# vivek87799/lightweight-human-pose-estimation.pytorch

Measured on AMD Instinct MI355X. Metric: frames/sec end-to-end (net+grouping) at 368px, higher is better.
Workload: dtype f32; 1 GPU; batch=1 per GPU, 368x656 frames, 1 refinement stage(s), fp32 convs / f32+f64 post, resident normalised NCHW input -> key-points + pose entries on host; 3 frame batch(es) in flight per GPU (3 engine stream(s), each step a complete pass); global_batch=1, parallelism=dp1 (frames sharded, no data-path collective), 3 stream(s) per GPU

## Files before the change

### lightweight-human-pose-estimation.pytorch_amd/csrc/capi.cpp

```cpp
#include <algorithm>
#include <cmath>
#include <cstdio>
#include <cstdlib>
#include <cstring>
#include <map>
#include <mutex>
#include <string>
#include <system_error>
#include <thread>
#include <vector>

#include "jpeg_host.h"
#include "lwp_internal.h"
#include "lwp_owners.h"

using namespace lwp;

struct lwp_context {
    int device = 0;
    Stream stream, post_own;
    hipStream_t post_stream = nullptr;
    int dtype = LWP_F32;
    Graph g;
    Tuning tune;
// ... 720 lines not shown
}
static inline int buf_level(const lwp_context* h, int buf) {
    const int nb = (int)h->g.bufs.size();
    return buf < 0 ? 0 : buf < nb ? h->g.bufs[buf].level : h->tp.bufs[buf - nb].level;
}

static int enqueue_layer(lwp_context* h, const Layer& l, const float* d_in, int N, int H, int W, float* const* d_outs_nchw,
                         const Layer* fold = nullptr, bool* folded = nullptr) {
    const bool h16 = h->dtype != LWP_F32;
    const int f16 = h->dtype == LWP_F16;
    const float* wts = h->blob(l.w_off);
    const float* bias = h->blob(l.b_off);
    int dh, dw;
    level_dims(H, W, buf_level(h, l.dst.buf), &dh, &dw);
    float* dst = buf_at(h, l.dst);
    char* vb = h->record_variants ? h->variant_buf : nullptr;
    if (vb) vb[0] = 0;
    if (l.kind == L_STEM) {
        StemParams p{d_in, wts, bias, dst, N, H, W, dh, dw, f16, h->d_zeros.as<float>()};
        p.tune = &h->tune; p.variant = vb;
        LAUNCH(h, KC_STEM, h16 ? launch_stem_bf16(p, h->stream) : launch_stem(p, h->stream));
    } else if (l.kind == L_DWPW) {
        int sh, sw;
        level_dims(H, W, buf_level(h, l.src.buf), &sh, &sw);
        DwPwParams p;
        p.in = buf_at(h, l.src); p.in_ld = l.src.ld; p.f16 = f16;
        p.dw_w = wts; p.pw_w = h->blob(l.w2_off); p.pw_b = h->blob(l.b2_off);
        p.out = dst; p.out_ld = l.dst.ld;
        p.res = l.res.buf >= 0 ? buf_at(h, l.res) : nullptr; p.res_ld = l.res.ld;
        p.zeros = h->d_zeros.as<float>();
        p.N = N; p.Hi = sh; p.Wi = sw; p.Ho = dh; p.Wo = dw; p.C = l.cin; p.cout = l.cout;
        p.stride = l.stride; p.dil = l.dil; p.act_dw = l.act; p.act_pw = l.act2;
        p.tune = &h->tune; p.variant = vb;
        LAUNCH(h, KC_PW, h16 ? launch_dwpw_bf16(p, h->stream) : launch_dwpw(p, h->stream));
    } else if (l.kind == L_DW) {
        int sh, sw;
        level_dims(H, W, buf_level(h, l.src.buf), &sh, &sw);
        DwParams p{buf_at(h, l.src), l.src.ld, wts, bias, dst, l.dst.ld, N, sh, sw, dh, dw, l.cin, l.stride, l.dil, l.act};
        p.tune = &h->tune; p.variant = vb;
        LAUNCH(h, KC_DW, launch_dw(p, h->stream));
    } else {
        GemmParams p;
        p.in = buf_at(h, l.src); p.in_ld = l.src.ld; p.f16 = f16;
        p.w = wts; p.bias = bias;
        p.wf = h16 ? nullptr : h->blob(l.w2_off);
        p.out = dst; p.out_ld = l.dst.ld;
        p.res = l.res.buf >= 0 ? buf_at(h, l.res) : nullptr; p.res_ld = l.res.ld;
        p.out_nchw = (l.out_index >= 0 && d_outs_nchw) ? d_outs_nchw[l.out_index] : nullptr;
        p.out_nchw2 = (l.out_index2 >= 0 && d_outs_nchw) ? d_outs_nchw[l.out_index2] : nullptr;
        p.out_split = l.out_split;
        p.zeros = h->d_zeros.as<float>();
        p.N = N; p.H = dh; p.W = dw;
        p.cin_pad = l.cin_pad; p.cout = l.cout; p.cout_pad = l.cout_pad; p.ks = l.ks; p.dil = l.dil; p.act = l.act;
        p.tune = &h->tune; p.variant = vb;
        if (fold) {
            p.w2 = h->blob(fold->w_off); p.bias2 = h->blob(fold->b_off);
            p.out2 = buf_at(h, fold->dst); p.out2_ld = fold->dst.ld; p.act2 = fold->act;
            p.fused2 = folded;
        }
        LAUNCH(h, l.ks == 1 ? KC_PW : KC_C3, h16 ? launch_gemm_bf16(p, h->stream) : launch_gemm(p, h->stream));
    }
    if (vb && h->cur_layer >= 0 && h->cur_layer < (int)h->variants.size()) h->variants[h->cur_layer] = vb;
    return LWP_OK;
}

static bool heads_pair_runs(const lwp_context* h, const Layer& a, const Layer& b, int64_t M) {
// ... 33 lines not shown
    return LWP_OK;
}

static int enqueue_forward(lwp_context* h, const std::vector<Layer>& ls, int begin, int end, const float* d_in, int N, int H, int W,
                           float* const* d_outs_nchw, bool retain = false) {
    int fh, fw;
    level_dims(H, W, 3, &fh, &fw);
    const int64_t M3 = (int64_t)N * fh * fw;
    int rc = LWP_OK;
    for (int i = begin; i < end && rc == LWP_OK; ++i) {
        h->cur_layer = i;
        const bool inside = i + 1 < end;
        if (inside && heads_pair_runs(h, ls[i], ls[i + 1], M3)) {
            if (retain) rc = enqueue_layer(h, ls[i], d_in, N, H, W, nullptr);
            if (!rc) rc = enqueue_heads_pair(h, ls[i], ls[i + 1], N, H, W, d_outs_nchw);
            ++i;
            continue;
        }
        if (retain && &ls == &h->tp.layers) {
            if (h->tp.dw_copy[i] >= 0) {
                rc = enqueue_dw_copy(h, ls[i], h->tp.dw_copy[i], N, H, W);
                if (rc) break;
            }
            if (h->tp.nores_copy[i] >= 0) {
                Layer c = ls[i];
                c.res = BufRef();
                c.dst.buf = h->tp.nores_copy[i]; c.dst.coff = 0;
                c.out_index = c.out_index2 = -1;
                rc = enqueue_layer(h, c, d_in, N, H, W, nullptr);
                if (rc) break;
            }
        }
        bool folded = false;
        rc = enqueue_layer(h, ls[i], d_in, N, H, W, d_outs_nchw, inside && ls[i].fuse == LWP_MARK_FOLD_NEXT_1X1 ? &ls[i + 1] : nullptr, &folded);
        if (!rc && folded) {
            if (h->record_variants && (size_t)i + 1 < h->variants.size()) h->variants[i + 1] = h->variants[i];
            ++i;
        }
    }
    h->cur_layer = -1;
    return rc;
}
static int enqueue_network(lwp_context* h, const float* d_in, int N, int H, int W, float* const* d_outs_nchw) {
    return enqueue_forward(h, h->g.layers, 0, (int)h->g.layers.size(), d_in, N, H, W, d_outs_nchw);
}

static int check_frame_shape(lwp_context* h, int N, int H, int W) {
    if (N <= 0 || H <= 0 || W <= 0) return fail(h, LWP_ERR_ARG, "bad frame shape");
    if (H < 8 || W < 8) return fail(h, LWP_ERR_ARG, "frame too small (H, W >= 8)");
    if (!h->weights_loaded) return fail(h, LWP_ERR_STATE, "weights not loaded (call lwp_load_weights first)");
    return LWP_OK;
}

static int stage_input(lwp_context* h, const float* in, int in_mem, size_t bytes, const float** d_in) {
    if (in_mem == LWP_MEM_DEVICE) { *d_in = in; return LWP_OK; }
    HIP_TRY(h, h->d_in.ensure(bytes));
    HIP_TRY(h, hipMemcpyAsync(h->d_in.as<float>(), in, bytes, hipMemcpyHostToDevice, h->stream));
    *d_in = h->d_in.as<float>();
    return LWP_OK;
}

extern "C" int lwp_forward(lwp_handle h, const float* in, int in_mem, int N, int H, int W, float* const* outs, int out_mem) {
    if (!h || !in || !outs) return fail(h, LWP_ERR_ARG, "null argument");
    int rc = check_frame_shape(h, N, H, W);
    if (rc) return rc;
    HIP_TRY(h, hipSetDevice(h->device));
    rc = ensure_activations(h, frames_per_pass(h, N, H, W), H, W);
    if (rc) return rc;
    if (in_mem == LWP_MEM_DEVICE || out_mem == LWP_MEM_DEVICE) { rc = order_in(h); if (rc) return rc; }
// ... 3948 lines not shown
```

### lightweight-human-pose-estimation.pytorch_amd/csrc/lwp_internal.h

```cpp
#pragma once
#include <hip/hip_runtime.h>
#include <stdint.h>
#include <algorithm>
#include <cstdio>
#include <string>
#include <vector>

#include "../../include/lwpose.h"

namespace lwp {

struct ParamSpec {
    std::string key;
    int64_t shape[4];
    int ndim;
    int role;
};
std::vector<ParamSpec> param_table(int nref, int C, int NH, int NP);

enum LayerKind { L_STEM = 0, L_DW = 1, L_GEMM = 2, L_DWPW = 3 };
enum Act { ACT_NONE = 0, ACT_RELU = 1, ACT_ELU = 2 };
enum KClass { KC_STEM = 0, KC_DW = 1, KC_PW = 2, KC_C3 = 3, KC_POST = 4, KC_OTHER = 5, KC_COUNT = 6 };

struct BufRef {
    int buf = -1;
    int coff = 0;
    int ld = 0;
};

struct WBlock {
    std::string conv_key;
    int out_off, in_off, cout, cin;
};

struct Layer {
    int kind = L_GEMM;
    std::string name;
    std::string conv_key;
    std::string bn_key;
    bool has_bias = false;
    int cin = 0, cout = 0, ks = 1, stride = 1, dil = 1, act = ACT_NONE;
    BufRef src, dst, res;
    int out_index = -1;
    int out_index2 = -1, out_split = 0;
    std::vector<WBlock> blocks;
    int64_t macs_per_pixel = 0;
    int fuse = LWP_MARK_NONE;
    size_t w_off = 0, b_off = 0;
    int cin_pad = 0, cout_pad = 0;
    std::string conv2_key, bn2_key;
    int act2 = ACT_NONE;
    size_t w2_off = 0, b2_off = 0;
};

struct BufSpec {
    int level;
    int channels;
    bool has_pad = false;
};

struct Graph {
    int nref, C, NH, NP;
    std::vector<BufSpec> bufs;
    std::vector<Layer> layers;
    size_t blob_floats = 0;
    int cat_buf = -1;
    int cat_channels = 0;
    int dtype = LWP_F32;
};
Graph build_graph(int nref, int C, int NH, int NP, bool fuse_dwpw, int dtype, bool merge_heads = true);

struct TrainPlan {
    std::vector<Layer> layers;
    std::vector<BufSpec> bufs;
    std::vector<int> cats;
    int cpm_conv = -1;
    int cpm_in = -1;
    int cut = -1;
    std::vector<int> dw_copy, nores_copy;
    enum { GRAD_ALWAYS = 0, GRAD_NEVER = 1, GRAD_ON_DEMAND = 2 };
    std::vector<char> grad_mode;
};
TrainPlan build_train_plan(const Graph& g, int scope = LWP_TRAIN_STAGES);
uint16_t f32_to_f16_rne(float f);
uint16_t f32_to_bf16_rne(float f);

struct HostTensor {
    const void* ptr;
    int64_t shape[4];
    int ndim;
};
std::string pack_weights(const Graph& g, const std::vector<std::string>& names,
                         const std::vector<HostTensor>& tensors, std::vector<float>& blob);

struct Tuning {
    int stem_ty = 0, stem_wl = -1, stem_debug = 0;
    int dw_tiled = -1, dw_cc = 0, dw_ph = 0;
    int dw_px = 0;
    int gemm_wp = -1;
    int gemm_debug = 0;
    bool has_c3 = false, has_pw = false; int c3[3] = {0, 0, 0}, pw[3] = {0, 0, 0};
    int dwpw_bm = 0, dwpw_nw = 0, dwpw_debug = 0, dwpwh_debug = 0;
    int dwpw_pipe = -1;
    int dwpw_lean = -1;
    int dwpw_tiled_wgs = 0;
    int dwpw_tiled = -1;
    int dwpw_pp_grid = 0;
    int dwpw_pp = -1;
    int heads_rm = 0;
    int gemmh_fold = -1;
    int gemmh_persist = -1, gemmh_ar_off = 0, gemmh_ar_force = 0, gemmh_debug = 0;
    bool has_gemmh_ar = false, has_gemmh = false; int gemmh_ar[4] = {0, 0, 0, 0}, gemmh[4] = {0, 0, 0, 0};
    int upsample_tiled = -1;
    int max_frames_per_pass = 0;
    int peak_tile = -1, pair_form = -1;
    int dwpw_lds_pad_kb = 0;
    int host_fetch_dma = -1;
    int ms_tx = 0;
    int ms_vec = -1;
    int ms_fused = -1;
    int heads_debug = 0;
    int heads_f32_lds = -1;
    int post_nchw = -1;
    int heads_f32_max_m = 0;
    int fuse_dwpw = -1, merge_heads = -1, fuse_heads = -1;
    int pre_batch_vec = -1;
    int post_stream = -1, post_generic = -1;
};
Tuning tuning_from_env();
const Tuning& default_tuning();
#ifdef __HIPCC__
__device__ __forceinline__ float relu_f(float v) { return v < 0.f ? 0.f : v; }
#endif
constexpr int kVariantCap = 64;
#define LWP_VARIANT(p, ...) do { if ((p).variant) snprintf((p).variant, lwp::kVariantCap, __VA_ARGS__); } while (0)

struct StemParams {
// ... 14 lines not shown
    int N, Hi, Wi, Ho, Wo, C, stride, dil, act;
    const Tuning* tune = nullptr; char* variant = nullptr;
};
struct GemmParams {
    const float* in; int in_ld;
    int f16 = 0;
    const float* w;
    const float* wf = nullptr;
    const float* bias;
    float* out; int out_ld;
    const float* res; int res_ld;
    float* out_nchw;
    float* out_nchw2 = nullptr;
    int out_split = 0;
    const float* zeros;
    int N, H, W, cin_pad, cout, cout_pad, ks, dil, act;
    int debug = 0;
    const Tuning* tune = nullptr; char* variant = nullptr;
    const void* w2 = nullptr; const float* bias2 = nullptr; void* out2 = nullptr; int out2_ld = 0, act2 = 0;
    bool* fused2 = nullptr;
};
struct DwPwParams {
    const float* in; int in_ld;
    int f16 = 0;
    const float* dw_w;
    const float* pw_w;
    const float* pw_b;
    float* out; int out_ld;
    const float* res; int res_ld;
    const float* zeros;
    int N, Hi, Wi, Ho, Wo, C, cout, stride, dil, act_dw, act_pw;
    int debug = 0;
    const Tuning* tune = nullptr; char* variant = nullptr;
};
bool dwpw_supported(int C, int cout);
hipError_t launch_dwpw(const DwPwParams& p, hipStream_t s);
hipError_t try_dwpw_tiled_f32(const DwPwParams& p, hipStream_t s, bool* used);
hipError_t try_dwpw_tiled_bf16(const DwPwParams& p, hipStream_t s, bool* used);
hipError_t launch_stem_bf16(const StemParams& p, hipStream_t s);
hipError_t launch_dwpw_bf16(const DwPwParams& p, hipStream_t s);
hipError_t launch_gemm_bf16(const GemmParams& p, hipStream_t s);
struct HeadsParams {
    const void* in; int in_ld;
    int f16 = 0;
    const void* w0; const float* b0;
    const float* w0f = nullptr;
    const void* w1; const float* b1;
    void* out; int out_ld;
    float* out_nchw; float* out_nchw2;
    int out_split, N, H, W, hidden, cout;
    const Tuning* tune = nullptr; char* variant = nullptr;
};
bool heads_bf16_supported(int cin_pad, int hidden, int cout_pad);
hipError_t launch_heads_bf16(const HeadsParams& p, hipStream_t s);
bool heads_f32_supported(int cin_pad, int hidden, int cout_pad, int64_t M, const Tuning* tune = nullptr);
hipError_t launch_heads_f32(const HeadsParams& p, hipStream_t s);
hipError_t launch_nchw_from_nhwc_bf16(const void* src, int src_ld, float* dst, int N, int HW, int C, hipStream_t s, bool f16 = false);
hipError_t launch_stem(const StemParams& p, hipStream_t s);
hipError_t launch_dw(const DwParams& p, hipStream_t s);
hipError_t launch_gemm(const GemmParams& p, hipStream_t s);

struct MapView {
    const float* base;
    int64_t ns, ys, xs, cs;
    int h, w;
};
struct PostCaps { int max_peaks = 2048, max_kpts = 128, max_conn = 4096, max_entries = 256; };
// ... 449 lines not shown
```

### lightweight-human-pose-estimation.pytorch_amd/csrc/net_graph.cpp

```cpp
#include <algorithm>
#include <cmath>
#include <cstring>
#include <map>

#include "lwp_internal.h"

namespace lwp {

static const int kBackbone[11][4] = {
    {32, 64, 1, 1},   {64, 128, 2, 1},  {128, 128, 1, 1}, {128, 256, 2, 1}, {256, 256, 1, 1}, {256, 512, 1, 1},
    {512, 512, 1, 2}, {512, 512, 1, 1}, {512, 512, 1, 1}, {512, 512, 1, 1}, {512, 512, 1, 1}};

static std::string fmt(const char* f, int a = 0, int b = 0) {
    char buf[128];
    snprintf(buf, sizeof buf, f, a, b);
    return buf;
}

static void add_conv(std::vector<ParamSpec>& t, const std::string& p, int cin, int cout, int k, int groups, bool bias) {
    ParamSpec w{p + ".weight", {cout, cin / groups, k, k}, 4, LWP_ROLE_CONV_W};
    t.push_back(w);
    if (bias) t.push_back(ParamSpec{p + ".bias", {cout, 1, 1, 1}, 1, LWP_ROLE_CONV_B});
}
static void add_bn(std::vector<ParamSpec>& t, const std::string& p, int c) {
// ... 54 lines not shown
        g.bufs.push_back(BufSpec{level, ch});
        return (int)g.bufs.size() - 1;
    }
    static BufRef ref(int buf, int ld, int coff = 0) {
        BufRef r;
        r.buf = buf; r.ld = ld; r.coff = coff;
        return r;
    }
    Layer& add(int kind, const std::string& name, const std::string& conv, const std::string& bn, bool bias,
               int cin, int cout, int ks, int stride, int dil, int act, BufRef src, BufRef dst) {
        Layer l;
        l.kind = kind; l.name = name; l.conv_key = conv; l.bn_key = bn; l.has_bias = bias;
        l.cin = cin; l.cout = cout; l.ks = ks; l.stride = stride; l.dil = dil; l.act = act;
        l.src = src; l.dst = dst;
        g.layers.push_back(l);
        return g.layers.back();
    }
};
}

static void mark_fusions(Graph& g) {
    std::vector<Layer>& ls = g.layers;
    auto ends_with = [](const std::string& s, const char* suf) { const size_t n = strlen(suf); return s.size() >= n && s.compare(s.size() - n, n, suf) == 0; };
    for (size_t i = 0; i + 1 < ls.size(); ++i) {
        Layer& a = ls[i];
        const Layer& b = ls[i + 1];
        if (ends_with(a.name, ".heads.0") && ends_with(b.name, ".heads.1") &&
            a.kind == L_GEMM && b.kind == L_GEMM && a.ks == 1 && b.ks == 1 && a.act == ACT_RELU && b.act == ACT_NONE &&
            a.res.buf < 0 && b.res.buf < 0 && a.out_index < 0 &&
            b.src.buf == a.dst.buf && b.src.coff == a.dst.coff && b.cin_pad == a.cout_pad && a.cout == a.cout_pad) {
            a.fuse = LWP_MARK_HEADS_PAIR;
            continue;
        }
        if (g.dtype == LWP_F32) continue;
        const bool later_reader = [&]() {
            for (size_t k = i + 2; k < ls.size(); ++k) {
                if ((ls[k].src.buf == a.dst.buf && ls[k].src.coff == a.dst.coff) || (ls[k].res.buf == a.dst.buf)) return true;
                if (ls[k].dst.buf == a.dst.buf) return false;
            }
            return false;
        }();
        if (a.kind == L_GEMM && a.ks == 3 && b.kind == L_GEMM && b.ks == 1 && b.src.buf == a.dst.buf && b.src.coff == a.dst.coff &&
            b.src.ld == a.dst.ld && b.res.buf < 0 && b.out_index < 0 && a.out_index < 0 && b.blocks.empty() && a.cout == 128 &&
            b.cin_pad == 128 && b.cout_pad == 128 && b.cout == 128 && !later_reader)
            a.fuse = LWP_MARK_FOLD_NEXT_1X1;
    }
}

Graph build_graph(int nref, int C, int NH, int NP, bool fuse_dwpw, int dtype, bool merge_heads) {
    Builder b;
    Graph& g = b.g;
    g.nref = nref; g.C = C; g.NH = NH; g.NP = NP; g.dtype = dtype;
    const bool h16 = dtype != LWP_F32;
    if (h16) fuse_dwpw = true;
    int s1 = b.new_buf(1, 32), d1 = b.new_buf(1, 32), p1 = b.new_buf(1, 64);
    int d2 = b.new_buf(2, 64), p2 = b.new_buf(2, 128), d3 = b.new_buf(2, 128), p3 = b.new_buf(2, 128);
    int X = b.new_buf(3, 512), Y = b.new_buf(3, 512);
    int S0 = b.new_buf(3, C), S1 = b.new_buf(3, C), S2 = b.new_buf(3, C);
    int catc = round_up(C + NH + NP, 64);
    int CAT = b.new_buf(3, catc);
    g.bufs[CAT].has_pad = true;
    const int H2 = b.new_buf(3, 1024 > 2 * C ? 1024 : 2 * C);
    g.cat_buf = CAT; g.cat_channels = catc;

    b.add(L_STEM, "model.0", "model.0.0", "model.0.1", false, 3, 32, 3, 2, 1, ACT_RELU, Builder::ref(-1, 3), Builder::ref(s1, 32));
    int src = s1, src_ld = 32;
    int dwbuf[11] = {d1, d2, d3, X, X, X, X, X, X, X, X};
    int pwbuf[11] = {p1, p2, p3, Y, Y, Y, Y, Y, Y, Y, Y};
    for (int i = 0; i < 11; ++i) {
        int cin = kBackbone[i][0], cout = kBackbone[i][1], st = kBackbone[i][2], dl = kBackbone[i][3];
        if (fuse_dwpw && dwpw_supported(cin, cout)) {
            const int dstb = (pwbuf[i] == src) ? (src == Y ? X : Y) : pwbuf[i];
            Layer& f = b.add(L_DWPW, fmt("model.%d.pw", i + 1), fmt("model.%d.0", i + 1), fmt("model.%d.1", i + 1), false, cin, cout, 3, st, dl,
                             ACT_RELU, Builder::ref(src, src_ld), Builder::ref(dstb, cout));
// ... 318 lines not shown
```

### lightweight-human-pose-estimation.pytorch_amd/csrc/net_kernels.hip

```cpp
#include <cstdio>
#include <cstdlib>

#include <type_traits>
#include "lwp_internal.h"

namespace lwp {

typedef float f32x4 __attribute__((ext_vector_type(4)));
typedef float f32x2 __attribute__((ext_vector_type(2)));
typedef float f32x16 __attribute__((ext_vector_type(16)));

__device__ __forceinline__ float elu_negative(float v) {
    const float p = v * (1.f + v * (0.5f + v * (1.f / 6.f + v * (1.f / 24.f + v * (1.f / 120.f + v * (1.f / 720.f + v * (1.f / 5040.f)))))));
    return v > -0.5f ? p : __expf(v) - 1.0f;
}
__device__ __forceinline__ float apply_act(float v, int act) {
    if (act == ACT_RELU) return relu_f(v);
    if (act == ACT_ELU) return v > 0.0f ? v : elu_negative(v);
    return v;
}

constexpr int ST_TX = 32;
template <bool BF16, int ST_TY, int PY = 1, int DBG = 0, bool WL = false, bool F16 = false>
__global__ void __launch_bounds__(ST_TY * ST_TX) stem_kernel(StemParams p) {
    typedef typename std::conditional<F16, _Float16, __bf16>::type h16;
    constexpr int NT = ST_TY * ST_TX;
    constexpr int TROWS = ST_TY * PY;
    constexpr int IR = 2 * TROWS + 1;
    constexpr int IQ = 18, ICP = IQ * 4;
    constexpr int OLD = BF16 ? 20 : 36;
    constexpr int IN_FLOATS = 3 * IR * ICP, OUT_FLOATS = NT * OLD;
    __shared__ __attribute__((aligned(16))) float smem[IN_FLOATS > OUT_FLOATS ? IN_FLOATS : OUT_FLOATS];
    float* s_in = smem;
    float* s_out = smem;
    __shared__ __attribute__((aligned(16))) float s_w[WL ? 27 * 32 : 4];
// ... 1016 lines not shown

struct GemmCfg { int bm, bn, ks; };

static hipError_t dispatch_gemm(const GemmParams& p, hipStream_t s, GemmCfg c) {
    const Tuning& T = p.tune ? *p.tune : default_tuning();
    const bool wp_set = T.gemm_wp >= 0;
    if (c.bm == 32 && !wp_set) {
        bool fits = false;
        hipError_t e = hipSuccess;
#define AR_CASE(BN_, KS_) if (c.bn == BN_ && c.ks == KS_) e = launch_gemm_ar_t<BN_, KS_>(p, s, &fits);
        AR_CASE(64, 1) AR_CASE(64, 2) AR_CASE(64, 4) AR_CASE(32, 4) AR_CASE(32, 8)
#undef AR_CASE
        if (fits) LWP_VARIANT(p, "gemm_ar<%d,%d,%d>", c.bn, c.ks, p.ks);
        if (e != hipSuccess || fits) return e;
    }
    if (c.bm == 32 && T.gemm_wp != 0) {
        LWP_VARIANT(p, "gemm_wp<%d,%d,%d>", c.bn, c.ks, p.ks);
#define WP_CASE(BN_, KS_) if (c.bn == BN_ && c.ks == KS_) return launch_gemm_wp_t<BN_, KS_>(p, s);
        WP_CASE(64, 1) WP_CASE(64, 2) WP_CASE(64, 4) WP_CASE(64, 8) WP_CASE(32, 4) WP_CASE(32, 8)
#undef WP_CASE
    }
    LWP_VARIANT(p, "gemm<%d,%d,%d,%d>", c.bm, c.bn, c.ks, p.ks);
#define GEMM_CASE(BM_, BN_, KS_) \
    if (c.bm == BM_ && c.bn == BN_ && c.ks == KS_) return launch_gemm_t<BM_, BN_, KS_>(p, s);
    GEMM_CASE(32, 64, 1) GEMM_CASE(32, 64, 2) GEMM_CASE(32, 64, 4)
    GEMM_CASE(64, 64, 1) GEMM_CASE(64, 64, 2) GEMM_CASE(64, 64, 4)
    GEMM_CASE(64, 128, 1) GEMM_CASE(64, 128, 2)
    GEMM_CASE(128, 128, 1)
    GEMM_CASE(32, 32, 4) GEMM_CASE(32, 32, 8)
#undef GEMM_CASE
    return hipErrorInvalidValue;
}

hipError_t launch_gemm(const GemmParams& p, hipStream_t s) {
    const int64_t M = (int64_t)p.N * p.H * p.W;
    const int nsteps = p.ks * p.ks * (p.cin_pad / BK);
    GemmCfg c{64, 64, 1};
    const Tuning& T = p.tune ? *p.tune : default_tuning();
    if (p.ks == 3 ? T.has_c3 : T.has_pw) {
        const int* v = p.ks == 3 ? T.c3 : T.pw;
        const GemmCfg o{v[0], v[1], v[2]};
        if (o.bn > 0 && (p.cout_pad % o.bn) == 0) return dispatch_gemm(p, s, o);
    }
    const int64_t t64 = ((M + 63) / 64) * (p.cout_pad / 64);
    const int64_t t32 = ((M + 31) / 32) * (p.cout_pad / 64);
    const int64_t t128 = (p.cout_pad % 128 == 0) ? ((M + 127) / 128) * (p.cout_pad / 128) : 0;
    const int64_t rounds128 = (t128 + 511) / 512;
    if (t128 >= 400 && (t128 >= 2048 || t128 * 5 >= rounds128 * 512 * 4)) {
        c = GemmCfg{128, 128, 1};
    } else if (t64 >= 400) {
        c = GemmCfg{64, 64, (t64 < 1024 && nsteps >= 8) ? 2 : 1};
    } else if (p.cout_pad == 64 && nsteps >= 16) {
        c = GemmCfg{32, 32, 8};
    } else {
        c = GemmCfg{32, 64, nsteps >= 4 ? 4 : (nsteps >= 2 ? 2 : 1)};
        if (t32 >= 1024 && c.ks > 2) c.ks = 2;
    }
    return dispatch_gemm(p, s, c);
}

constexpr int DWPW_F32_APAD = 4;
constexpr int DWPW_LEAN_DEFAULT = 1;
template <int BM, int NW, int DBG = 0, int ACT = -1, int LEAN = 0>
__global__ void __launch_bounds__(NW * 64) __attribute__((amdgpu_waves_per_eu(LEAN ? 6 : 0, LEAN ? 6 : 0))) dwpw_kernel(DwPwParams p) {
    static_assert(!LEAN || (BM == 16 && NW == 16 && DBG == 0), "the lean phase 1 is written for one item per thread");
    const int act_dw = ACT >= 0 ? ACT : p.act_dw, act_pw = ACT >= 0 ? ACT : p.act_pw;
    constexpr int NT = NW * 64;
    constexpr int RT = BM / 16;
    extern __shared__ __attribute__((aligned(16))) float dsm[];
    const int ldA = p.C + DWPW_F32_APAD;
    float* At = dsm;

    const int tid = threadIdx.x, lane = tid & 63;
    const int wave = blockIdx.y * NW + (tid >> 6);
    const int wave_u = __builtin_amdgcn_readfirstlane(wave);
    const __amdgpu_buffer_rsrc_t wrsrc = __builtin_amdgcn_make_buffer_rsrc((void*)p.pw_w, 0, 0x7fffffff, 0x00020000);
    const int nwt = gridDim.y * NW;
    const int r16 = lane & 15, q = lane >> 4;
    const int64_t M = (int64_t)p.N * p.Ho * p.Wo;
    int bid = blockIdx.x;
    if (gridDim.y == 1 && !(DBG & 8)) {
        const int nwg = gridDim.x, qq = nwg >> 3, rem = nwg & 7, xcd = bid & 7;
        bid = (xcd < rem ? xcd * (qq + 1) : rem * (qq + 1) + (xcd - rem) * qq) + (bid >> 3);
    }
    const int64_t m0 = (int64_t)bid * BM;
    const int nsteps = p.C / 32;

#ifndef DWPW_PF
#define DWPW_PF 2
#endif
    constexpr int PF = DWPW_PF;
    f32x4 bw[PF][4];
    auto load_b = [&](int step, f32x4* dst) {
        const unsigned soff = (unsigned)(step * nwt + wave_u) * 4096u;
#pragma unroll
        for (int j = 0; j < 4; ++j)
            dst[j] = __builtin_bit_cast(f32x4, __builtin_amdgcn_raw_buffer_load_b128(wrsrc, lane * 16 + j * 1024, soff, 0));
    };
// ... 193 lines not shown
    __syncthreads();

    f32x4 acc[RT][2];
#pragma unroll
    for (int a = 0; a < RT; ++a) { acc[a][0] = f32x4{0.f, 0.f, 0.f, 0.f}; acc[a][1] = f32x4{0.f, 0.f, 0.f, 0.f}; }
    const float* a_lane = At + r16 * ldA + 4 * q;
    auto one = [&](int step, auto P_) {
        constexpr int P = decltype(P_)::value;
        const int nxt = step + PF - 1 < nsteps ? step + PF - 1 : nsteps - 1;
        if (!(DBG & 2)) load_b(nxt, bw[(P + PF - 1) % PF]);
        __builtin_amdgcn_sched_barrier(0);
        if (DBG & 4) return;
        const f32x4* bcur = bw[P];
#pragma unroll
        for (int u = 0; u < 2; ++u) {
            f32x4 av[RT];
#pragma unroll
            for (int a = 0; a < RT; ++a) av[a] = *(const f32x4*)(a_lane + a * 16 * ldA + step * 32 + 16 * u);
#pragma unroll
            for (int j = 0; j < 4; ++j) {
#pragma unroll
                for (int t = 0; t < 2; ++t) {
                    const int v = u * 8 + j * 2 + t;
                    const float b = bcur[v >> 2][v & 3];
#pragma unroll
                    for (int a = 0; a < RT; ++a) acc[a][t] = __builtin_amdgcn_mfma_f32_16x16x4f32(b, av[a][j], acc[a][t], 0, 0, 0);
                }
            }
        }
    };
    f32x4 bias[2];
#pragma unroll
    for (int t = 0; t < 2; ++t) bias[t] = *(const f32x4*)(p.pw_b + wave * 32 + t * 16 + 4 * q);
    int s0 = 0;
    for (; s0 + PF <= nsteps; s0 += PF) {
        one(s0, std::integral_constant<int, 0>{});
        if (PF > 1) one(s0 + 1, std::integral_constant<int, 1 % PF>{});
        if (PF > 2) one(s0 + 2, std::integral_constant<int, 2 % PF>{});
    }
    if (s0 < nsteps) { one(s0, std::integral_constant<int, 0>{}); ++s0; }
    if (PF > 2 && s0 < nsteps) { one(s0, std::integral_constant<int, 1 % PF>{}); ++s0; }
    f32x4 resv[RT][2];
    if (p.res) {
#pragma unroll
        for (int t = 0; t < 2; ++t)
#pragma unroll
            for (int a = 0; a < RT; ++a) {
                const int64_t m = m0 + a * 16 + r16;
                resv[a][t] = m < M ? *(const f32x4*)(p.res + m * p.res_ld + wave * 32 + t * 16 + 4 * q) : f32x4{0.f, 0.f, 0.f, 0.f};
            }
    }
#pragma unroll
    for (int t = 0; t < 2; ++t) {
        const int n = wave * 32 + t * 16 + 4 * q;
#pragma unroll
        for (int a = 0; a < RT; ++a) {
            const int64_t m = m0 + a * 16 + r16;
            if (m < M) {
                f32x4 v = acc[a][t] + bias[t];
                v.x = apply_act(v.x, act_pw); v.y = apply_act(v.y, act_pw);
                v.z = apply_act(v.z, act_pw); v.w = apply_act(v.w, act_pw);
                if (p.res) v += resv[a][t];
                *(f32x4*)(p.out + m * p.out_ld + n) = v;
            }
        }
    }
}

template <int BM, int NW, int DBG = 0, int ACT = -1>
static hipError_t launch_dwpw_t(const DwPwParams& p, hipStream_t s) {
    const int64_t M = (int64_t)p.N * p.Ho * p.Wo;
    const size_t lds = (size_t)BM * (p.C + DWPW_F32_APAD) * sizeof(float);
    if ((int64_t)p.N * p.Hi * p.Wi * p.in_ld * 4 >= (1ll << 31)) return hipErrorInvalidValue;
    const int nsplit = (p.cout / 32) / NW;
    if constexpr (BM == 16 && NW == 16 && DBG == 0 && ACT == ACT_RELU) {
        const Tuning& T = p.tune ? *p.tune : default_tuning();
        if ((T.dwpw_lean < 0 ? DWPW_LEAN_DEFAULT : T.dwpw_lean) != 0 && p.C <= 512) {
            hipLaunchKernelGGL((dwpw_kernel<BM, NW, DBG, ACT, 1>), dim3((unsigned)((M + BM - 1) / BM), nsplit), dim3(NW * 64), lds, s, p);
            return hipGetLastError();
        }
    }
    static LdsAttrOnce attr;
    if (lds > 48 * 1024) {
        hipError_t e = attr.ensure((const void*)dwpw_kernel<BM, NW, DBG, ACT>, 160 * 1024);
        if (e != hipSuccess) return e;
    }
    hipLaunchKernelGGL((dwpw_kernel<BM, NW, DBG, ACT>), dim3((unsigned)((M + BM - 1) / BM), nsplit), dim3(NW * 64), lds, s, p);
    return hipGetLastError();
}

template <int C>
__global__ void __launch_bounds__(1024) dwpw_pipe_kernel(DwPwParams p, int ntiles) {
    constexpr int BM = 32, NT = 1024, RT = BM / 16, NSTEP = C / 32;
    constexpr int ldA = C + DWPW_F32_APAD;
    constexpr int CG = C / 4;
    constexpr int PAR = NT / CG;
    constexpr int NIT = BM / PAR;
    static_assert(NIT * 4 == NSTEP, "one pixel per four K steps");
    extern __shared__ __attribute__((aligned(16))) float dsm[];
    float* Wd = dsm + 2 * BM * ldA;
    const int tid = threadIdx.x, lane = tid & 63;
    const int wave_u = __builtin_amdgcn_readfirstlane(tid >> 6);
    const int r16 = lane & 15, q = lane >> 4;
    const int M32 = p.N * p.Ho * p.Wo;
    const int G = gridDim.x;
    int bid = blockIdx.x;
    {
        const int qq = G >> 3, rem = G & 7, xcd = bid & 7;
        bid = (xcd < rem ? xcd * (qq + 1) : rem * (qq + 1) + (xcd - rem) * qq) + (bid >> 3);
    }
// ... 137 lines not shown
}

hipError_t launch_dwpw(const DwPwParams& p_in, hipStream_t s) {
    const DwPwParams& p = p_in;
    {
        bool used = false;
        hipError_t e = try_dwpw_tiled_f32(p, s, &used);
        if (e != hipSuccess || used) return e;
        e = try_dwpw_pipe(p, s, &used);
        if (e != hipSuccess || used) return e;
    }
    const int64_t M = (int64_t)p.N * p.Ho * p.Wo;
    const int nw = p.cout / 32;
    int bm = 16;
    if (M / 32 >= 450) bm = 32;
    if (M / 64 >= 900) bm = 64;
    if (bm == 64 && nw >= 16) bm = 32;
    int nw_wg = nw;
    const Tuning& T = p.tune ? *p.tune : default_tuning();
    if (T.dwpw_bm) bm = T.dwpw_bm;
    if (T.dwpw_nw > 0 && T.dwpw_nw < nw && nw % T.dwpw_nw == 0) nw_wg = T.dwpw_nw;
    if (bm > 64) bm = 64;
    while (bm > 16 && (size_t)bm * (p.C + DWPW_F32_APAD) * sizeof(float) > 150 * 1024) bm >>= 1;
    LWP_VARIANT(p, "dwpw<%d,%d>", bm, nw_wg);
#ifdef LWP_ABLATION
    const int d = T.dwpw_debug;
#define DP_DBG(BM_, NW_, D_) if (bm == BM_ && nw_wg == NW_ && d == D_) return launch_dwpw_t<BM_, NW_, D_>(p, s);
#define DP_DBGS(BM_, NW_) DP_DBG(BM_, NW_, 1) DP_DBG(BM_, NW_, 2) DP_DBG(BM_, NW_, 3) DP_DBG(BM_, NW_, 4) DP_DBG(BM_, NW_, 6) DP_DBG(BM_, NW_, 7) DP_DBG(BM_, NW_, 8)
    DP_DBGS(16, 16) DP_DBGS(16, 8) DP_DBGS(16, 4)
#undef DP_DBGS
#undef DP_DBG
#endif
    const bool relu = p.act_dw == ACT_RELU && p.act_pw == ACT_RELU;
#define DP_CASE(BM_, NW_) if (bm == BM_ && nw_wg == NW_) return relu ? launch_dwpw_t<BM_, NW_, 0, ACT_RELU>(p, s) : launch_dwpw_t<BM_, NW_>(p, s);
    DP_CASE(16, 2) DP_CASE(32, 2) DP_CASE(64, 2)
    DP_CASE(16, 4) DP_CASE(32, 4) DP_CASE(64, 4)
    DP_CASE(16, 8) DP_CASE(32, 8) DP_CASE(64, 8)
    DP_CASE(16, 16) DP_CASE(32, 16) DP_CASE(64, 16)
#undef DP_CASE
    return hipErrorInvalidValue;
}

constexpr int HX_LD = 32 + 4, HX_QS = 32 * HX_LD;
template <int NW, int DBG = 0>
__global__ void __launch_bounds__(NW * 64) heads_f32_kernel(HeadsParams p) {
    static_assert(NW == 8, "the reduction maps the 8 waves onto 2 pixel blocks x 4 output tiles");
    extern __shared__ __attribute__((aligned(16))) float hsm[];
    float* const xs = hsm + NW * 2 * 4 * 64 * 4;
    const int tid = threadIdx.x, lane = tid & 63;
    const int wave = __builtin_amdgcn_readfirstlane(tid >> 6);
    const int i16 = lane & 15, q = lane >> 4;
    const int M = p.N * p.H * p.W;
    int bid = blockIdx.x;
    {
        const int nwg = gridDim.x, qq = nwg >> 3, rem = nwg & 7, xcd = bid & 7;
        bid = (xcd < rem ? xcd * (qq + 1) : rem * (qq + 1) + (xcd - rem) * qq) + (bid >> 3);
    }
    const int nheads = p.out_split > 0 ? 2 : 1;
    const int head = nheads == 2 ? (bid & 1) : 0;
    const int ptile = nheads == 2 ? (bid >> 1) : bid;
    int mm[2];
    bool mok[2];
#pragma unroll
    for (int x = 0; x < 2; ++x) { mm[x] = ptile * 32 + x * 16 + i16; mok[x] = mm[x] < M; }
    const float* in = (const float*)p.in;
    const __amdgpu_buffer_rsrc_t xr = __builtin_amdgcn_make_buffer_rsrc((void*)in, 0, (int)((int64_t)M * p.in_ld * 4), 0x00020000);
    const __amdgpu_buffer_rsrc_t w0fr = __builtin_amdgcn_make_buffer_rsrc((void*)p.w0f, 0, p.hidden * 128 * 4, 0x00020000);
// ... 328 lines not shown
        const size_t lds2 = (size_t)(2 * HL_HC * HL_LD0 + 2 * 64 * HL_LD1 + p.hidden) * sizeof(float);
        static LdsAttrOnce attr;
        hipError_t e = attr.ensure((const void*)heads_f32_lds_kernel<PT>, 96 * 1024);
        if (e != hipSuccess) return e;
        LWP_VARIANT(p, "heads_f32_lds<%d>", PT);
        hipLaunchKernelGGL(heads_f32_lds_kernel<PT>, dim3((unsigned)((M + 64 * PT - 1) / (64 * PT))), dim3(256), lds2, s, p);
        return hipGetLastError();
    }
    const size_t lds = ((size_t)NW * 2 * 4 * 64 * 4 + 4 * HX_QS) * sizeof(float);
    const unsigned nheads = p.out_split > 0 ? 2u : 1u;
    if (p.out_split < 0 || p.out_split >= p.cout || p.hidden % 32 || !p.w0f) return hipErrorInvalidValue;
    const unsigned grid = (unsigned)((M + 31) / 32) * nheads;
    LWP_VARIANT(p, "heads_f32<%d>", NW);
#ifdef LWP_ABLATION
    const int d = (p.tune ? *p.tune : default_tuning()).heads_debug;
#define HD_DBG(D_) if (d == D_) return launch_heads_f32_i<NW, D_>(p, s, grid, lds);
    HD_DBG(1) HD_DBG(2) HD_DBG(4) HD_DBG(8) HD_DBG(7) HD_DBG(15)
#undef HD_DBG
#endif
    return launch_heads_f32_i<NW, 0>(p, s, grid, lds);
}

const Tuning& default_tuning() { static const Tuning t; return t; }
Tuning tuning_from_env() {
    Tuning t;
    auto geti = [](const char* name, int* dst) { const char* e = getenv(name); if (e && e[0]) *dst = atoi(e); };
    auto digit = [](const char* name, int* dst) { const char* e = getenv(name); if (e && e[0]) *dst = e[0] - '0'; };
    geti("LWP_STEM_TY", &t.stem_ty); digit("LWP_STEM_WL", &t.stem_wl); geti("LWP_STEM_DEBUG", &t.stem_debug);
    digit("LWP_DW_TILED", &t.dw_tiled); geti("LWP_DW_CC", &t.dw_cc); geti("LWP_DW_PH", &t.dw_ph); geti("LWP_DW_PX", &t.dw_px);
    digit("LWP_GEMM_WP", &t.gemm_wp);
    if (const char* e = getenv("LWP_GEMM_C3")) t.has_c3 = sscanf(e, "%d,%d,%d", &t.c3[0], &t.c3[1], &t.c3[2]) == 3;
    if (const char* e = getenv("LWP_GEMM_PW")) t.has_pw = sscanf(e, "%d,%d,%d", &t.pw[0], &t.pw[1], &t.pw[2]) == 3;
    geti("LWP_DWPW_BM", &t.dwpw_bm); geti("LWP_DWPW_NW", &t.dwpw_nw); geti("LWP_DWPW_DEBUG", &t.dwpw_debug); geti("LWP_DWPWH_DEBUG", &t.dwpwh_debug);
    digit("LWP_DWPW_PIPE", &t.dwpw_pipe); digit("LWP_DWPW_LEAN", &t.dwpw_lean);
    digit("LWP_DWPW_TILED", &t.dwpw_tiled); geti("LWP_DWPW_TILED_WGS", &t.dwpw_tiled_wgs);
    digit("LWP_DWPW_PP", &t.dwpw_pp); geti("LWP_DWPW_PP_GRID", &t.dwpw_pp_grid);
    geti("LWP_HEADS_RM", &t.heads_rm);
    digit("LWP_GEMMH_PERSIST", &t.gemmh_persist); digit("LWP_GEMMH_FOLD", &t.gemmh_fold);
    if (const char* e = getenv("LWP_GEMMH_AR")) {
        if (e[0] == '0' && e[1] == 0) t.gemmh_ar_off = 1;
        else t.has_gemmh_ar = sscanf(e, "%d,%d,%d,%d", &t.gemmh_ar[0], &t.gemmh_ar[1], &t.gemmh_ar[2], &t.gemmh_ar[3]) == 4;
    }
    if (const char* e = getenv("LWP_GEMMH_AR_FORCE")) t.gemmh_ar_force = e[0] == '1';
    geti("LWP_GEMMH_DEBUG", &t.gemmh_debug); geti("LWP_GEMM_DEBUG", &t.gemm_debug);
    if (const char* e = getenv("LWP_GEMMH")) t.has_gemmh = sscanf(e, "%d,%d,%d,%d", &t.gemmh[0], &t.gemmh[1], &t.gemmh[2], &t.gemmh[3]) == 4;
    digit("LWP_UPSAMPLE_TILED", &t.upsample_tiled);
    digit("LWP_PEAK_TILE", &t.peak_tile); digit("LWP_PAIR_FORM", &t.pair_form); digit("LWP_POST_NCHW", &t.post_nchw); digit("LWP_HEADS_F32_LDS", &t.heads_f32_lds); digit("LWP_MS_FUSED", &t.ms_fused); digit("LWP_MS_VEC", &t.ms_vec); geti("LWP_MS_TX", &t.ms_tx); digit("LWP_HOST_FETCH_DMA", &t.host_fetch_dma); geti("LWP_DWPW_LDS_PAD", &t.dwpw_lds_pad_kb);
    geti("LWP_HEADS_F32_MAXM", &t.heads_f32_max_m); geti("LWP_HEADS_DEBUG", &t.heads_debug);
    geti("LWP_MAX_FRAMES_PER_PASS", &t.max_frames_per_pass);
    digit("LWP_FUSE_DWPW", &t.fuse_dwpw); digit("LWP_MERGE_HEADS", &t.merge_heads); digit("LWP_FUSE_HEADS", &t.fuse_heads);
    digit("LWP_PRE_BATCH_VEC", &t.pre_batch_vec); digit("LWP_POST_STREAM", &t.post_stream); digit("LWP_POST_GENERIC", &t.post_generic);
    return t;
}

__global__ void __launch_bounds__(256) nchw_from_nhwc_kernel(const float* src, int src_ld, float* dst, int N, int HW, int C) {
    const int64_t total = (int64_t)N * C * HW;
    const int64_t idx = (int64_t)blockIdx.x * blockDim.x + threadIdx.x;
    if (idx >= total) return;
    const int pix = (int)(idx % HW);
    const int64_t t = idx / HW;
    const int c = (int)(t % C);
    const int n = (int)(t / C);
    dst[idx] = src[((int64_t)n * HW + pix) * src_ld + c];
}
hipError_t launch_nchw_from_nhwc(const float* src, int src_ld, float* dst, int N, int HW, int C, hipStream_t s) {
    const int64_t total = (int64_t)N * C * HW;
    hipLaunchKernelGGL(nchw_from_nhwc_kernel, dim3((unsigned)((total + 255) / 256)), dim3(256), 0, s, src, src_ld, dst, N, HW, C);
// ... 5 lines not shown
```

Measured before the change: 2819 frames/s.

## Fold following 1x1 conv into lean fp32 depthwise-pointwise kernel for 512->128 layers

In fp32 mode, marks DWPW layers (ReLU, 512 out) followed by a 1x1 ReLU conv to 128 channels, and folds that second conv into the lean dwpw kernel. The first conv's output tile goes through LDS and is multiplied by the 512x128 weights with MFMA, split across waves and reduced through LDS. This avoids writing and re-reading the 512-channel intermediate and saves a launch. It also adds a compile-time ELU specialisation for dwpw kernels. The risks are extra LDS and register pressure in the lean kernel, and a reduction order that differs from the standalone gemm.

```diff
diff --git a/lightweight-human-pose-estimation.pytorch_amd/csrc/capi.cpp b/lightweight-human-pose-estimation.pytorch_amd/csrc/capi.cpp
--- a/lightweight-human-pose-estimation.pytorch_amd/csrc/capi.cpp
+++ b/lightweight-human-pose-estimation.pytorch_amd/csrc/capi.cpp
@@ -776,6 +776,11 @@
         p.N = N; p.Hi = sh; p.Wi = sw; p.Ho = dh; p.Wo = dw; p.C = l.cin; p.cout = l.cout;
         p.stride = l.stride; p.dil = l.dil; p.act_dw = l.act; p.act_pw = l.act2;
         p.tune = &h->tune; p.variant = vb;
+        if (fold && !h16) {
+            p.w2f = h->blob(fold->w2_off); p.bias2 = h->blob(fold->b_off);
+            p.out2 = buf_at(h, fold->dst); p.out2_ld = fold->dst.ld;
+            p.fused2 = folded;
+        }
         LAUNCH(h, KC_PW, h16 ? launch_dwpw_bf16(p, h->stream) : launch_dwpw(p, h->stream));
     } else if (l.kind == L_DW) {
         int sh, sw;
@@ -875,9 +880,10 @@
             }
         }
         bool folded = false;
-        rc = enqueue_layer(h, ls[i], d_in, N, H, W, d_outs_nchw, inside && ls[i].fuse == LWP_MARK_FOLD_NEXT_1X1 ? &ls[i + 1] : nullptr, &folded);
+        const bool offer = inside && (ls[i].fuse == LWP_MARK_FOLD_NEXT_1X1 || (ls[i].takes_next_1x1 && !retain));
+        rc = enqueue_layer(h, ls[i], d_in, N, H, W, d_outs_nchw, offer ? &ls[i + 1] : nullptr, &folded);
         if (!rc && folded) {
-            if (h->record_variants && (size_t)i + 1 < h->variants.size()) h->variants[i + 1] = h->variants[i];
+            if (h->record_variants && (size_t)i + 1 < h->variants.size()) h->variants[i + 1] = ls[i].kind == L_DWPW ? std::string(kDwPwFoldSumsAs) : h->variants[i];
             ++i;
         }
     }
diff --git a/lightweight-human-pose-estimation.pytorch_amd/csrc/lwp_internal.h b/lightweight-human-pose-estimation.pytorch_amd/csrc/lwp_internal.h
--- a/lightweight-human-pose-estimation.pytorch_amd/csrc/lwp_internal.h
+++ b/lightweight-human-pose-estimation.pytorch_amd/csrc/lwp_internal.h
@@ -46,6 +46,7 @@
     std::vector<WBlock> blocks;
     int64_t macs_per_pixel = 0;
     int fuse = LWP_MARK_NONE;
+    bool takes_next_1x1 = false;
     size_t w_off = 0, b_off = 0;
     int cin_pad = 0, cout_pad = 0;
     std::string conv2_key, bn2_key;
@@ -103,6 +104,8 @@
     int dwpw_bm = 0, dwpw_nw = 0, dwpw_debug = 0, dwpwh_debug = 0;
     int dwpw_pipe = -1;
     int dwpw_lean = -1;
+    int fold_align = -1;
+    int dwpw_elu_ct = -1;
     int dwpw_tiled_wgs = 0;
     int dwpw_tiled = -1;
     int dwpw_pp_grid = 0;
@@ -183,7 +186,10 @@
     int N, Hi, Wi, Ho, Wo, C, cout, stride, dil, act_dw, act_pw;
     int debug = 0;
     const Tuning* tune = nullptr; char* variant = nullptr;
-};
+    const float* w2f = nullptr; const float* bias2 = nullptr; float* out2 = nullptr; int out2_ld = 0;
+    bool* fused2 = nullptr;
+};
+constexpr const char* kDwPwFoldSumsAs = "gemm_ar<64,4,1>";
 bool dwpw_supported(int C, int cout);
 hipError_t launch_dwpw(const DwPwParams& p, hipStream_t s);
 hipError_t try_dwpw_tiled_f32(const DwPwParams& p, hipStream_t s, bool* used);
diff --git a/lightweight-human-pose-estimation.pytorch_amd/csrc/net_graph.cpp b/lightweight-human-pose-estimation.pytorch_amd/csrc/net_graph.cpp
--- a/lightweight-human-pose-estimation.pytorch_amd/csrc/net_graph.cpp
+++ b/lightweight-human-pose-estimation.pytorch_amd/csrc/net_graph.cpp
@@ -110,7 +110,6 @@
             a.fuse = LWP_MARK_HEADS_PAIR;
             continue;
         }
-        if (g.dtype == LWP_F32) continue;
         const bool later_reader = [&]() {
             for (size_t k = i + 2; k < ls.size(); ++k) {
                 if ((ls[k].src.buf == a.dst.buf && ls[k].src.coff == a.dst.coff) || (ls[k].res.buf == a.dst.buf)) return true;
@@ -118,6 +117,14 @@
             }
             return false;
         }();
+        if (g.dtype == LWP_F32) {
+            if (a.kind == L_DWPW && a.act == ACT_RELU && a.act2 == ACT_RELU && a.res.buf < 0 && a.out_index < 0 && a.cout == 512 &&
+                b.kind == L_GEMM && b.ks == 1 && b.has_bias && b.act == ACT_RELU && b.res.buf < 0 && b.out_index < 0 && b.blocks.empty() &&
+                b.src.buf == a.dst.buf && b.src.coff == a.dst.coff && b.src.ld == a.dst.ld && b.cin == a.cout && b.cin_pad == a.cout &&
+                b.cout == 128 && b.cout_pad == 128 && !later_reader)
+                a.takes_next_1x1 = true;
+            continue;
+        }
         if (a.kind == L_GEMM && a.ks == 3 && b.kind == L_GEMM && b.ks == 1 && b.src.buf == a.dst.buf && b.src.coff == a.dst.coff &&
             b.src.ld == a.dst.ld && b.res.buf < 0 && b.out_index < 0 && a.out_index < 0 && b.blocks.empty() && a.cout == 128 &&
             b.cin_pad == 128 && b.cout_pad == 128 && b.cout == 128 && !later_reader)
diff --git a/lightweight-human-pose-estimation.pytorch_amd/csrc/net_kernels.hip b/lightweight-human-pose-estimation.pytorch_amd/csrc/net_kernels.hip
--- a/lightweight-human-pose-estimation.pytorch_amd/csrc/net_kernels.hip
+++ b/lightweight-human-pose-estimation.pytorch_amd/csrc/net_kernels.hip
@@ -1,6 +1,8 @@
 #include <cstdio>
 #include <cstdlib>
-
+#include <cstring>
+
+#include <algorithm>
 #include <type_traits>
 #include "lwp_internal.h"
 
@@ -1083,38 +1085,53 @@
     return hipErrorInvalidValue;
 }
 
+static GemmCfg gemm_heuristic(int64_t M, int cout_pad, int nsteps) {
+    GemmCfg c{64, 64, 1};
+    const int64_t t64 = ((M + 63) / 64) * (cout_pad / 64);
+    const int64_t t32 = ((M + 31) / 32) * (cout_pad / 64);
+    const int64_t t128 = (cout_pad % 128 == 0) ? ((M + 127) / 128) * (cout_pad / 128) : 0;
+    const int64_t rounds128 = (t128 + 511) / 512;
+    if (t128 >= 400 && (t128 >= 2048 || t128 * 5 >= rounds128 * 512 * 4)) {
+        c = GemmCfg{128, 128, 1};
+    } else if (t64 >= 400) {
+        c = GemmCfg{64, 64, (t64 < 1024 && nsteps >= 8) ? 2 : 1};
+    } else if (cout_pad == 64 && nsteps >= 16) {
+        c = GemmCfg{32, 32, 8};
+    } else {
+        c = GemmCfg{32, 64, nsteps >= 4 ? 4 : (nsteps >= 2 ? 2 : 1)};
+        if (t32 >= 1024 && c.ks > 2) c.ks = 2;
+    }
+    return c;
+}
+
 hipError_t launch_gemm(const GemmParams& p, hipStream_t s) {
     const int64_t M = (int64_t)p.N * p.H * p.W;
     const int nsteps = p.ks * p.ks * (p.cin_pad / BK);
-    GemmCfg c{64, 64, 1};
     const Tuning& T = p.tune ? *p.tune : default_tuning();
     if (p.ks == 3 ? T.has_c3 : T.has_pw) {
         const int* v = p.ks == 3 ? T.c3 : T.pw;
         const GemmCfg o{v[0], v[1], v[2]};
         if (o.bn > 0 && (p.cout_pad % o.bn) == 0) return dispatch_gemm(p, s, o);
     }
-    const int64_t t64 = ((M + 63) / 64) * (p.cout_pad / 64);
-    const int64_t t32 = ((M + 31) / 32) * (p.cout_pad / 64);
-    const int64_t t128 = (p.cout_pad % 128 == 0) ? ((M + 127) / 128) * (p.cout_pad / 128) : 0;
-    const int64_t rounds128 = (t128 + 511) / 512;
-    if (t128 >= 400 && (t128 >= 2048 || t128 * 5 >= rounds128 * 512 * 4)) {
-        c = GemmCfg{128, 128, 1};
-    } else if (t64 >= 400) {
-        c = GemmCfg{64, 64, (t64 < 1024 && nsteps >= 8) ? 2 : 1};
-    } else if (p.cout_pad == 64 && nsteps >= 16) {
-        c = GemmCfg{32, 32, 8};
-    } else {
-        c = GemmCfg{32, 64, nsteps >= 4 ? 4 : (nsteps >= 2 ? 2 : 1)};
-        if (t32 >= 1024 && c.ks > 2) c.ks = 2;
-    }
-    return dispatch_gemm(p, s, c);
+    return dispatch_gemm(p, s, gemm_heuristic(M, p.cout_pad, nsteps));
+}
+
+static bool gemm_1x1_to_128_is_ar_64_4(const Tuning& T, int64_t M, int cin, int out_ld) {
+    if (T.has_pw || T.gemm_wp >= 0 || T.gemm_debug) return false;
+    const GemmCfg c = gemm_heuristic(M, 128, cin / BK);
+    if (c.bm != 32 || c.bn != 64 || c.ks != 4) return false;
+    return M * cin * 4 < (1ll << 31) && ((M - 1) * out_ld + 128) * 4 < (1ll << 31);
 }
 
 constexpr int DWPW_F32_APAD = 4;
 constexpr int DWPW_LEAN_DEFAULT = 1;
-template <int BM, int NW, int DBG = 0, int ACT = -1, int LEAN = 0>
+constexpr int DWPW_FOLD_DEFAULT = 1;
+constexpr int DWPW_FOLD_N = 128;
+constexpr int DWPW_FOLD_LDR = DWPW_FOLD_N + 4;
+template <int BM, int NW, int DBG = 0, int ACT = -1, int LEAN = 0, int FOLD = 0>
 __global__ void __launch_bounds__(NW * 64) __attribute__((amdgpu_waves_per_eu(LEAN ? 6 : 0, LEAN ? 6 : 0))) dwpw_kernel(DwPwParams p) {
     static_assert(!LEAN || (BM == 16 && NW == 16 && DBG == 0), "the lean phase 1 is written for one item per thread");
+    static_assert(!FOLD || (LEAN && ACT == ACT_RELU), "the folded 1x1 is written for the lean ReLU form");
     const int act_dw = ACT >= 0 ? ACT : p.act_dw, act_pw = ACT >= 0 ? ACT : p.act_pw;
     constexpr int NT = NW * 64;
     constexpr int RT = BM / 16;
@@ -1374,6 +1391,11 @@
     f32x4 bias[2];
 #pragma unroll
     for (int t = 0; t < 2; ++t) bias[t] = *(const f32x4*)(p.pw_b + wave * 32 + t * 16 + 4 * q);
+    f32x4 bias2 = f32x4{0.f, 0.f, 0.f, 0.f};
+    if constexpr (FOLD) {
+        const __amdgpu_buffer_rsrc_t b2rsrc = __builtin_amdgcn_make_buffer_rsrc((void*)p.bias2, 0, DWPW_FOLD_N * 4, 0x00020000);
+        bias2 = __builtin_bit_cast(f32x4, __builtin_amdgcn_raw_buffer_load_b128(b2rsrc, (tid & 31) * 16, 0, 0));
+    }
     int s0 = 0;
     for (; s0 + PF <= nsteps; s0 += PF) {
         one(s0, std::integral_constant<int, 0>{});
@@ -1382,6 +1404,74 @@
     }
     if (s0 < nsteps) { one(s0, std::integral_constant<int, 0>{}); ++s0; }
     if (PF > 2 && s0 < nsteps) { one(s0, std::integral_constant<int, 1 % PF>{}); ++s0; }
+    if constexpr (FOLD) {
+        constexpr unsigned OOB = 0x80000000u;
+        constexpr int NU = 8;
+        typedef unsigned u32x4 __attribute__((ext_vector_type(4)));
+        const int g2 = wave_u >> 2, pr = wave_u & 3;
+        const int h2 = q & 1;
+        const bool hi = q >= 2;
+        const __amdgpu_buffer_rsrc_t w2rsrc = __builtin_amdgcn_make_buffer_rsrc((void*)p.w2f, 0, 512 * DWPW_FOLD_N * 4, 0x00020000);
+        f32x4 w2[2][4];
+        auto load_w2 = [&](int i, f32x4* dst) {
+            const unsigned soff = (unsigned)((((g2 + 4 * (i >> 1)) * 4 + pr) * 4 + 2 * (i & 1)) * 1024);
+#pragma unroll
+            for (int sl = 0; sl < 2; ++sl)
+#pragma unroll
+                for (int t = 0; t < 2; ++t)
+                    dst[sl * 2 + t] = __builtin_bit_cast(f32x4, __builtin_amdgcn_raw_buffer_load_b128(w2rsrc, (h2 * 32 + 16 * t + r16) * 16 + sl * 1024, soff, 0));
+        };
+        load_w2(0, w2[0]);
+        f32x4 v[2];
+#pragma unroll
+        for (int t = 0; t < 2; ++t) {
+            v[t] = acc[0][t] + bias[t];
+            v[t].x = relu_f(v[t].x); v[t].y = relu_f(v[t].y); v[t].z = relu_f(v[t].z); v[t].w = relu_f(v[t].w);
+        }
+        __syncthreads();
+#pragma unroll
+        for (int t = 0; t < 2; ++t) *(f32x4*)(At + r16 * ldA + wave_u * 32 + t * 16 + 4 * q) = v[t];
+        __syncthreads();
+        f32x4 acc2[2] = {f32x4{0.f, 0.f, 0.f, 0.f}, f32x4{0.f, 0.f, 0.f, 0.f}};
+        const float* x_lane = At + r16 * ldA + 4 * h2;
+        auto one2 = [&](int i, auto P_) {
+            constexpr int P = decltype(P_)::value;
+            load_w2(i + 1 < NU ? i + 1 : NU - 1, w2[P ^ 1]);
+            __builtin_amdgcn_sched_barrier(0);
+            const int kb = (g2 + 4 * (i >> 1)) * 32 + 16 * (i & 1);
+#pragma unroll
+            for (int sl = 0; sl < 2; ++sl) {
+                const f32x4 xv = *(const f32x4*)(x_lane + kb + 8 * sl);
+                const float x0 = hi ? xv.y : xv.x, x1 = hi ? xv.w : xv.z;
+                const f32x4 wa = w2[P][sl * 2], wb = w2[P][sl * 2 + 1];
+                acc2[0] = __builtin_amdgcn_mfma_f32_16x16x4f32(hi ? wa.y : wa.x, x0, acc2[0], 0, 0, 0);
+                acc2[1] = __builtin_amdgcn_mfma_f32_16x16x4f32(hi ? wb.y : wb.x, x0, acc2[1], 0, 0, 0);
+                acc2[0] = __builtin_amdgcn_mfma_f32_16x16x4f32(hi ? wa.w : wa.z, x1, acc2[0], 0, 0, 0);
+                acc2[1] = __builtin_amdgcn_mfma_f32_16x16x4f32(hi ? wb.w : wb.z, x1, acc2[1], 0, 0, 0);
+            }
+        };
+        for (int i = 0; i < NU; i += 2) {
+            one2(i, std::integral_constant<int, 0>{});
+            one2(i + 1, std::integral_constant<int, 1>{});
+        }
+        __syncthreads();
+        float* red = dsm;
+#pragma unroll
+        for (int t = 0; t < 2; ++t) *(f32x4*)(red + (g2 * 16 + r16) * DWPW_FOLD_LDR + pr * 32 + 16 * t + 4 * q) = acc2[t];
+        __syncthreads();
+        if (tid < 16 * DWPW_FOLD_N / 4) {
+            const int pix = tid >> 5, c4 = (tid & 31) * 4;
+            f32x4 o = *(const f32x4*)(red + pix * DWPW_FOLD_LDR + c4);
+#pragma unroll
+            for (int gg = 1; gg < 4; ++gg) o += *(const f32x4*)(red + (gg * 16 + pix) * DWPW_FOLD_LDR + c4);
+            o += bias2;
+            o.x = relu_f(o.x); o.y = relu_f(o.y); o.z = relu_f(o.z); o.w = relu_f(o.w);
+            const int M32 = (int)M, m = (int)m0 + pix;
+            const __amdgpu_buffer_rsrc_t orsrc = __builtin_amdgcn_make_buffer_rsrc((void*)p.out2, 0, ((M32 - 1) * p.out2_ld + DWPW_FOLD_N) * 4, 0x00020000);
+            __builtin_amdgcn_raw_buffer_store_b128(__builtin_bit_cast(u32x4, o), orsrc, m < M32 ? (unsigned)(m * p.out2_ld + c4) * 4u : OOB, 0, 0);
+        }
+        return;
+    }
     f32x4 resv[RT][2];
     if (p.res) {
 #pragma unroll
@@ -1418,6 +1508,15 @@
     if constexpr (BM == 16 && NW == 16 && DBG == 0 && ACT == ACT_RELU) {
         const Tuning& T = p.tune ? *p.tune : default_tuning();
         if ((T.dwpw_lean < 0 ? DWPW_LEAN_DEFAULT : T.dwpw_lean) != 0 && p.C <= 512) {
+            if (p.fused2 && p.w2f && p.bias2 && p.out2 && (T.fold_align < 0 ? DWPW_FOLD_DEFAULT : T.fold_align) != 0 && p.C == 512 && p.cout == 512 &&
+                nsplit == 1 && !p.res && p.out2_ld >= DWPW_FOLD_N && (p.out2_ld & 3) == 0 && (((uintptr_t)p.out2) & 15) == 0 &&
+                M * p.out2_ld * 4 < (1ll << 31) && gemm_1x1_to_128_is_ar_64_4(T, M, p.cout, p.out2_ld)) {
+                const size_t lds2 = std::max(lds, (size_t)4 * 16 * DWPW_FOLD_LDR * sizeof(float));
+                *p.fused2 = true;
+                if (p.variant) { const size_t n = strlen(p.variant); snprintf(p.variant + n, kVariantCap - n, "+1x1"); }
+                hipLaunchKernelGGL((dwpw_kernel<BM, NW, DBG, ACT, 1, 1>), dim3((unsigned)((M + BM - 1) / BM), nsplit), dim3(NW * 64), lds2, s, p);
+                return hipGetLastError();
+            }
             hipLaunchKernelGGL((dwpw_kernel<BM, NW, DBG, ACT, 1>), dim3((unsigned)((M + BM - 1) / BM), nsplit), dim3(NW * 64), lds, s, p);
             return hipGetLastError();
         }
@@ -1621,7 +1720,8 @@
 #undef DP_DBG
 #endif
     const bool relu = p.act_dw == ACT_RELU && p.act_pw == ACT_RELU;
-#define DP_CASE(BM_, NW_) if (bm == BM_ && nw_wg == NW_) return relu ? launch_dwpw_t<BM_, NW_, 0, ACT_RELU>(p, s) : launch_dwpw_t<BM_, NW_>(p, s);
+    const bool elu = p.act_dw == ACT_ELU && p.act_pw == ACT_ELU && T.dwpw_elu_ct != 0;
+#define DP_CASE(BM_, NW_) if (bm == BM_ && nw_wg == NW_) return relu ? launch_dwpw_t<BM_, NW_, 0, ACT_RELU>(p, s) : elu ? launch_dwpw_t<BM_, NW_, 0, ACT_ELU>(p, s) : launch_dwpw_t<BM_, NW_>(p, s);
     DP_CASE(16, 2) DP_CASE(32, 2) DP_CASE(64, 2)
     DP_CASE(16, 4) DP_CASE(32, 4) DP_CASE(64, 4)
     DP_CASE(16, 8) DP_CASE(32, 8) DP_CASE(64, 8)
@@ -2016,7 +2116,7 @@
     if (const char* e = getenv("LWP_GEMM_C3")) t.has_c3 = sscanf(e, "%d,%d,%d", &t.c3[0], &t.c3[1], &t.c3[2]) == 3;
     if (const char* e = getenv("LWP_GEMM_PW")) t.has_pw = sscanf(e, "%d,%d,%d", &t.pw[0], &t.pw[1], &t.pw[2]) == 3;
     geti("LWP_DWPW_BM", &t.dwpw_bm); geti("LWP_DWPW_NW", &t.dwpw_nw); geti("LWP_DWPW_DEBUG", &t.dwpw_debug); geti("LWP_DWPWH_DEBUG", &t.dwpwh_debug);
-    digit("LWP_DWPW_PIPE", &t.dwpw_pipe); digit("LWP_DWPW_LEAN", &t.dwpw_lean);
+    digit("LWP_DWPW_PIPE", &t.dwpw_pipe); digit("LWP_DWPW_LEAN", &t.dwpw_lean); digit("LWP_FOLD_ALIGN", &t.fold_align); digit("LWP_DWPW_ELU_CT", &t.dwpw_elu_ct);
     digit("LWP_DWPW_TILED", &t.dwpw_tiled); geti("LWP_DWPW_TILED_WGS", &t.dwpw_tiled_wgs);
     digit("LWP_DWPW_PP", &t.dwpw_pp); geti("LWP_DWPW_PP_GRID", &t.dwpw_pp_grid);
     geti("LWP_HEADS_RM", &t.heads_rm);
```

Result: no change. 2840 frames/s (median of 4 runs) (+0.8%).
